# bmds-lab/Crackling

Measured on AMD Instinct MI355X. Metric: guides/sec (whole node) + achieved HBM GB/s, 20bp/<=4mm ISSL scan, higher is better.
Workload: dtype u32

## Files before the change

crackling_amd/csrc/issl_kernels.hip:

```cpp
#include <hip/hip_runtime.h>

#include <algorithm>
#include <type_traits>
#include <cstdio>

#include "issl_device.hpp"

namespace issl {

#define ISSL_CFD_QUAL __constant__
#include "cfd_tables.inc"


__device__ __forceinline__ void short_kernel_priority() { __builtin_amdgcn_s_setprio(3); }

__host__ __device__ inline uint32_t gather_even16(uint32_t x)
{
    x &= 0x55555555u;
    x = (x | (x >> 1)) & 0x33333333u;
    x = (x | (x >> 2)) & 0x0F0F0F0Fu;
    x = (x | (x >> 4)) & 0x00FF00FFu;
    x = (x | (x >> 8)) & 0x0000FFFFu;
    return x;
}
// ... 1657 lines not shown
}

__global__ __launch_bounds__(256) void k_prefix_of_sums(uint32_t *__restrict__ sums, uint32_t n_blocks)
{
    short_kernel_priority();
    __shared__ uint64_t lds[256];
    uint64_t carry = 0;
    for (uint32_t base = 0; base < n_blocks; base += 256) {
        const uint32_t i = base + threadIdx.x;
        const uint64_t val = i < n_blocks ? sums[i] : 0;
        uint64_t total;
        const uint64_t ex = block_exclusive_scan(val, lds, &total);
        if (i < n_blocks) sums[i] = static_cast<uint32_t>(carry + ex);
        carry += total;
    }
}

__global__ __launch_bounds__(256) void k_prefix_apply(const uint32_t *__restrict__ in, uint32_t n,
                                                      const uint32_t *__restrict__ sums, uint32_t *__restrict__ out,
                                                      uint32_t *__restrict__ big, Counters *__restrict__ counters,
                                                      uint32_t slot_hits)
{
    short_kernel_priority();
    __shared__ uint64_t lds[256];
    const uint32_t base = blockIdx.x * kScanChunk + threadIdx.x * 8u;
    uint32_t val[8];
    uint64_t s = 0;
    uint32_t nb = 0;
    for (uint32_t i = 0; i < 8; ++i) {
        const uint32_t c = (base + i < n) ? in[base + i] : 0u;
        nb += c > kReplayLds;
        val[i] = grouped_hits(c, slot_hits);
        s += val[i];
    }
    if (nb != 0u) {
        uint32_t at = atomicAdd(&counters->n_big, nb);
        for (uint32_t i = 0; i < 8; ++i)
            if (base + i < n && in[base + i] > kReplayLds) big[at++] = base + i;
    }
    uint64_t run = block_exclusive_scan(s, lds, nullptr) + sums[blockIdx.x];
    for (uint32_t i = 0; i < 8; ++i) {
        if (base + i < n) out[base + i] = static_cast<uint32_t>(run);
        run += val[i];
    }
}

__global__ __launch_bounds__(1024) void k_prefix_single(const uint32_t *__restrict__ in, uint32_t n,
                                                        uint32_t *__restrict__ out, uint32_t *__restrict__ big,
                                                        Counters *__restrict__ counters, uint32_t slot_hits)
{
    short_kernel_priority();
    if (slot_hits >= kReplayLds && counters->overflowed == 0u) return;
    __shared__ uint32_t wave_sum[16], wave_big[16];
    const uint32_t lane = threadIdx.x & 63u, wave = threadIdx.x >> 6;
    const uint32_t per = ((n + 1023u) / 1024u + 3u) & ~3u;
    const uint32_t i0 = threadIdx.x * per;
    uint32_t s = 0, b = 0;
    for (uint32_t k = 0; k < per; k += 4) {
        const uint32_t i = i0 + k;
        uint4 q = make_uint4(0, 0, 0, 0);
        if (i + 3 < n) q = *reinterpret_cast<const uint4 *>(in + i);
        else { if (i < n) q.x = in[i]; if (i + 1 < n) q.y = in[i + 1]; if (i + 2 < n) q.z = in[i + 2]; }
        s += grouped_hits(q.x, slot_hits) + grouped_hits(q.y, slot_hits) + grouped_hits(q.z, slot_hits) + grouped_hits(q.w, slot_hits);
        b += (q.x > kReplayLds) + (q.y > kReplayLds) + (q.z > kReplayLds) + (q.w > kReplayLds);
    }
    uint32_t x = s, xb = b;
    for (uint32_t d = 1; d < 64; d <<= 1) {
        const uint32_t y = __shfl_up(x, d, 64), yb = __shfl_up(xb, d, 64);
        if (lane >= d) { x += y; xb += yb; }
    }
    if (lane == 63) { wave_sum[wave] = x; wave_big[wave] = xb; }
    __syncthreads();
    uint32_t run = x - s, brun = xb - b;
    for (uint32_t wv = 0; wv < wave; ++wv) { run += wave_sum[wv]; brun += wave_big[wv]; }
    if (threadIdx.x == 1023u) counters->n_big = brun + b;
    for (uint32_t k = 0; k < per; k += 4) {
        const uint32_t i = i0 + k;
        if (i >= n) break;
        uint4 q = make_uint4(0, 0, 0, 0);
        if (i + 3 < n) q = *reinterpret_cast<const uint4 *>(in + i);
        else { q.x = in[i]; if (i + 1 < n) q.y = in[i + 1]; if (i + 2 < n) q.z = in[i + 2]; }
        const uint32_t ex = grouped_hits(q.x, slot_hits), ey = grouped_hits(q.y, slot_hits), ez = grouped_hits(q.z, slot_hits),
                       ew = grouped_hits(q.w, slot_hits);
        const uint4 o = make_uint4(run, run + ex, run + ex + ey, run + ex + ey + ez);
        if (i + 3 < n) *reinterpret_cast<uint4 *>(out + i) = o;
        else { out[i] = o.x; if (i + 1 < n) out[i + 1] = o.y; if (i + 2 < n) out[i + 2] = o.z; }
        run += ex + ey + ez + ew;
        if (q.x > kReplayLds) big[brun++] = i;
        if (q.y > kReplayLds) big[brun++] = i + 1;
        if (q.z > kReplayLds) big[brun++] = i + 2;
        if (q.w > kReplayLds) big[brun++] = i + 3;
    }
}

__global__ __launch_bounds__(kChunkRecs) void k_group_scatter(const uint64_t *__restrict__ raw,
                                                              const uint32_t *__restrict__ raw_used,
                                                              const Counters *__restrict__ counters, uint32_t cap_chunks,
                                                              const uint32_t *__restrict__ gcount,
                                                              const uint32_t *__restrict__ goff,
                                                              const uint32_t *__restrict__ rank,
                                                              const double2 *__restrict__ pay,
                                                              uint64_t *__restrict__ sorted, double2 *__restrict__ terms,
                                                              uint32_t slot_hits)
{
    short_kernel_priority();
    if (slot_hits >= kReplayLds && counters->n_big == 0u) return;
    uint32_t n_chunks = counters->raw_chunks;
    if (n_chunks > cap_chunks) n_chunks = cap_chunks;
    for (uint32_t chunk = blockIdx.x; chunk < n_chunks; chunk += gridDim.x) {
        const uint64_t *recs = raw + static_cast<uint64_t>(chunk) * kChunkRecs;
        const uint32_t t = threadIdx.x + 1u;
        const uint64_t slot = static_cast<uint64_t>(chunk) * (kChunkRecs - 1u) + (threadIdx.x < kChunkRecs - 1u ? threadIdx.x : kChunkRecs - 2u);
        const uint64_t key = recs[t < kChunkRecs ? t : 0u];
        const uint32_t my_rank = rank[slot];
        const double2 my_pay = pay[slot];
        const uint32_t used = raw_used[chunk];
        if (t >= used || t >= kChunkRecs || key == kDeadKey) continue;
        const uint32_t guide = static_cast<uint32_t>(key >> kKeyGuideShift);
        const uint32_t to = goff[guide] + my_rank;
        sorted[to] = key;
        if (gcount[guide] <= kMidHits) terms[to] = my_pay;
    }
}

void launch_group_hits(const Workspace &ws, uint32_t n, void *stream_)
{
    if (ws.lean_tail) return;
    hipStream_t stream = static_cast<hipStream_t>(stream_);
    const uint32_t m = n + 1;
    if (m <= (1u << 18)) {
        hipLaunchKernelGGL(k_prefix_single, dim3(1), dim3(1024), 0, stream, ws.gcount, m, ws.goff, ws.gcur_big,
                           ws.counters, ws.slot_hits);
    } else {
        const uint32_t blocks = (m + kScanChunk - 1) / kScanChunk;
        hipLaunchKernelGGL(k_prefix_block_sums, dim3(blocks), dim3(256), 0, stream, ws.gcount, m, ws.blocksum, ws.slot_hits);
        hipLaunchKernelGGL(k_prefix_of_sums, dim3(1), dim3(256), 0, stream, ws.blocksum, blocks);
        hipLaunchKernelGGL(k_prefix_apply, dim3(blocks), dim3(256), 0, stream, ws.gcount, m, ws.blocksum, ws.goff,
                           ws.gcur_big, ws.counters, ws.slot_hits);
    }
    hipLaunchKernelGGL(k_group_scatter, dim3(kTailGrid), dim3(kChunkRecs), 0, stream, ws.raw, ws.raw_used, ws.counters,
                       static_cast<uint32_t>(ws.cap_chunks), ws.gcount, ws.goff, ws.rank, reinterpret_cast<const double2 *>(ws.pay),
                       ws.sorted, reinterpret_cast<double2 *>(ws.terms), ws.slot_hits);
}



__device__ inline void wave_sort(uint64_t *data, uint32_t n)
{
    if (n < 2) return;
    uint32_t np = 1;
    while (np < n) np <<= 1;
    for (uint32_t k = 2; k <= np; k <<= 1) {
        for (uint32_t j = k >> 1; j > 0; j >>= 1) {
            for (uint32_t t = threadIdx.x; t < (np >> 1); t += blockDim.x) {
                const uint32_t i = ((t & ~(j - 1u)) << 1) | (t & (j - 1u));
                const uint32_t l = (j == (k >> 1)) ? (i ^ (k - 1u)) : (i | j);
                if (l < n) {
                    const uint64_t a = data[i], b = data[l];
                    if (a > b) { data[i] = b; data[l] = a; }
                }
            }
            __syncthreads();
        }
    }
}

__device__ inline double bcast_f64(double x, int lane)
{
    const uint64_t u = __double_as_longlong(x);
    const uint32_t lo = __builtin_amdgcn_readlane(static_cast<uint32_t>(u), lane);
    const uint32_t hi = __builtin_amdgcn_readlane(static_cast<uint32_t>(u >> 32), lane);
    return __longlong_as_double((static_cast<uint64_t>(hi) << 32) | lo);
}

__device__ __forceinline__ bool accumulate_chunk(double mit_term, double cfd_term, uint32_t cnt, const ScoreParams &p,
                                                 uint32_t lane, double &tot_mit, double &tot_cfd, uint32_t &kept,
                                                 const double2 *chunk_lds)
{
    auto passes = [&](double m, double c) {
        if (p.method == ISSL_METHOD_AND) return m > p.maximum_sum && c > p.maximum_sum;
        if (p.method == ISSL_METHOD_OR) return m > p.maximum_sum || c > p.maximum_sum;
        if (p.method == ISSL_METHOD_AVG) return ((m + c) / 2.0) > p.maximum_sum;
        if (p.method == ISSL_METHOD_MIT) return m > p.maximum_sum;
        if (p.method == ISSL_METHOD_CFD) return c > p.maximum_sum;
        return false;
    };
    {
        double tm = tot_mit, tc = tot_cfd;
        for (uint32_t l0 = 0; l0 < cnt; l0 += 8) {
#pragma unroll
            for (uint32_t l = 0; l < 8; ++l) {
                const double2 t = chunk_lds[l0 + l];
                tm += t.x;
                tc += t.y;
            }
        }
        const bool grows = __ballot(lane < cnt && !(mit_term >= 0.0 && cfd_term >= 0.0)) == 0ull;
        if (grows && !passes(tm, tc)) {
            kept += cnt;
            tot_mit = tm;
            tot_cfd = tc;
            return false;
        }
    }
    double tm = tot_mit, tc = tot_cfd, mine_m = 0.0, mine_c = 0.0;
    for (uint32_t l0 = 0; l0 < cnt; l0 += 8) {
#pragma unroll
        for (uint32_t l = 0; l < 8; ++l) {
            const double2 t = chunk_lds[l0 + l];
            tm += t.x;
            tc += t.y;
            if (lane == l0 + l) { mine_m = tm; mine_c = tc; }
        }
    }
    const bool exit_here = passes(mine_m, mine_c);
    const uint64_t exits = __ballot(exit_here && lane < cnt);
    if (exits != 0ull) {
        const int first = __builtin_ctzll(exits);
        kept += static_cast<uint32_t>(first) + 1u;
        tot_mit = bcast_f64(mine_m, first);
        tot_cfd = bcast_f64(mine_c, first);
        return true;
    }
    kept += cnt;
    tot_mit = tm;
    tot_cfd = tc;
    return false;
}

struct HitTerms {
    double mit, cfd;
    issl_hit rec;
};

__device__ inline HitTerms hit_terms(const ImageView &v, uint64_t gsig, uint32_t g, uint64_t key, bool calc_mit,
                                     bool calc_cfd, bool want_id)
{
    HitTerms t;
    t.mit = 0.0;
    t.cfd = 0.0;
    const uint64_t low = (1ull << v.slice_width) - 1ull;
    const uint32_t slice = static_cast<uint32_t>(key >> kKeySliceShift) & kKeySliceMask;
    uint32_t pos = static_cast<uint32_t>(key);
    const uint32_t bucket = (slice << v.slice_width) + static_cast<uint32_t>((gsig >> (v.slice_width * slice)) & low);
    const uint64_t at = v.bucket_start[bucket] + pos;
    uint32_t id = 0, occ;
    uint64_t ot;
    if (v.srec || v.sid) {
        id = pos;
        const uint64_t site = v.sites[id];
        ot = site & kSigMask;
        occ = static_cast<uint32_t>(site >> 40);
        if (occ == kOccSaturated) occ = v.site_occ[id];
        pos = 0;
        if (want_id && v.entries) {
            const uint64_t *list = v.entries + v.bucket_start[bucket];
            uint64_t lo = 0, hi = v.bucket_start[bucket + 1] - v.bucket_start[bucket];
            while (lo < hi) {
                const uint64_t mid = (lo + hi) >> 1;
                if (static_cast<uint32_t>(list[mid]) < id) lo = mid + 1; else hi = mid;
            }
            pos = static_cast<uint32_t>(lo);
        } else if (want_id) {
            const uint32_t *ss = v.sub_start + static_cast<uint64_t>(bucket) * 257u;
            const uint64_t first = static_cast<uint64_t>(v.tile_first[bucket]) * kTileCands;
            for (uint32_t w = 0; w < 256u; ++w) {
                uint32_t lo = ss[w], hi = ss[w + 1];
                const uint32_t s0 = lo;
                while (lo < hi) {
                    const uint32_t mid = (lo + hi) >> 1;
                    const uint32_t there = v.srec ? v.srec[first + mid].id : v.sid[first + mid];
                    if (there < id) lo = mid + 1; else hi = mid;
                }
                pos += lo - s0;
            }
        }
    } else if (v.occ8) {
        ot = candidate_signature(v, bucket, v.tile_first[bucket] + (pos >> 11), pos & (kTileCands - 1u));
        occ = v.occ8[at];
        if (occ == 255u || want_id) {
            const uint64_t e = v.entries[at];
            id = static_cast<uint32_t>(e);
            occ = static_cast<uint32_t>(e >> 32);
        }
    } else {
        const uint64_t e = v.entries[at];
        id = static_cast<uint32_t>(e);
        occ = static_cast<uint32_t>(e >> 32);
        ot = v.esig ? v.esig[at] : v.sites[id];
    }
    int dist;
    score_terms(v, gsig, ot, occ, calc_mit, calc_cfd, t.mit, t.cfd, dist);
    t.rec.guide = g; t.rec.slice = slice; t.rec.pos = pos; t.rec.id = id;
    t.rec.dist = static_cast<uint32_t>(dist); t.rec.occ = occ;
    return t;
}

__global__ __launch_bounds__(64, 8) void k_replay(ImageView v, Workspace ws, const uint64_t *__restrict__ guides,
                                               uint32_t n, ScoreParams p, double *__restrict__ out_mit,
                                               double *__restrict__ out_cfd, uint32_t *__restrict__ out_kept,
                                               issl_hit *__restrict__ out_hits)
{
    short_kernel_priority();
    __shared__ uint64_t keys[kReplayLds];
    __shared__ __attribute__((aligned(16))) double2 ord[64];
    const bool calc_mit = p.method == ISSL_METHOD_MIT || p.method == ISSL_METHOD_AND || p.method == ISSL_METHOD_OR ||
                          p.method == ISSL_METHOD_AVG;
    const bool calc_cfd = p.method == ISSL_METHOD_CFD || p.method == ISSL_METHOD_AND || p.method == ISSL_METHOD_OR ||
                          p.method == ISSL_METHOD_AVG;
    const uint32_t lane = threadIdx.x;
    if (blockIdx.x == 0 && lane == 0 && ws.counters->overflowed != 0u) atomicOr(&ws.sticky[0], ws.lean_tail ? 6u : 4u);

    for (uint32_t g = blockIdx.x; g < n; g += gridDim.x) {
        const uint32_t h = ws.gcount[g];
        if (h > kReplayLds) continue;
        const bool slots = ws.slot_hits >= kReplayLds;
        const uint32_t h0 = slots ? 0u : ws.goff[g];
        const SlotRec *__restrict__ srec = ws.slots + static_cast<uint64_t>(g) * ws.slot_hits;
        const uint64_t *__restrict__ skeys = ws.sorted + h0;
        const double2 *__restrict__ sterms = reinterpret_cast<const double2 *>(ws.terms) + h0;
        auto key_of = [&](uint32_t i) { return slots ? srec[i].key : skeys[i]; };
        auto terms_of = [&](uint32_t i) { return slots ? *reinterpret_cast<const double2 *>(&srec[i].mit) : sterms[i]; };
        const uint64_t gsig = guides[g];
        double tot_mit = 0.0, tot_cfd = 0.0;
        uint32_t kept = 0;
        bool stop = false;

        auto accumulate = [&](double mit_term, double cfd_term, uint32_t cnt) {
            stop = accumulate_chunk(mit_term, cfd_term, cnt, p, lane, tot_mit, tot_cfd, kept, ord);
        };

        if (h <= 64) {
            uint64_t key = ~0ull;
            double2 mine = make_double2(0.0, 0.0);
            issl_hit rec{};
            if (lane < h) {
                key = key_of(lane);
                mine = terms_of(lane);
                if (out_hits) rec = hit_terms(v, gsig, g, key, calc_mit, calc_cfd, true).rec;
            }
            uint32_t rank = 0;
            for (uint32_t j = 0; j < h; ++j) {
                const uint32_t klo = __builtin_amdgcn_readlane(static_cast<uint32_t>(key), static_cast<int>(j));
                const uint32_t khi = __builtin_amdgcn_readlane(static_cast<uint32_t>(key >> 32), static_cast<int>(j));
                const uint64_t other = (static_cast<uint64_t>(khi) << 32) | klo;
                rank += (other < key) ? 1u : 0u;
            }
            if (lane < h) {
                ord[rank] = mine;
                if (out_hits) out_hits[h0 + rank] = rec;
            } else {
                ord[lane] = make_double2(0.0, 0.0);
            }
            __syncthreads();
            const double2 t = ord[lane];
            accumulate(t.x, t.y, h);
        } else {
            uint64_t *data = keys;
            for (uint32_t i = lane; i < h; i += 64) keys[i] = ((key_of(i) & ((1ull << kKeyGuideShift) - 1ull)) << 9) | i;
            __syncthreads();
            wave_sort(data, h);
            __syncthreads();
            for (uint32_t base = 0; base < h && !stop; base += 64) {
                const uint32_t idx = base + lane;
                double2 mine = make_double2(0.0, 0.0);
                if (idx < h) {
                    const uint64_t sv = data[idx];
                    mine = terms_of(static_cast<uint32_t>(sv & 511ull));
                    if (out_hits)
                        out_hits[h0 + idx] = hit_terms(v, gsig, g, (static_cast<uint64_t>(g) << kKeyGuideShift) | (sv >> 9), calc_mit, calc_cfd, true).rec;
                }
                __syncthreads();
                ord[lane] = mine;
                __syncthreads();
                accumulate(mine.x, mine.y, (h - base < 64u) ? h - base : 64u);
            }
        }
        if (lane == 0) {
            out_mit[g] = 10000.0 / (100.0 + tot_mit);
            out_cfd[g] = 10000.0 / (100.0 + tot_cfd);
            if (out_kept) out_kept[g] = kept;
        }
        __syncthreads();
    }
}

constexpr uint32_t kMidSlice = 1024;
constexpr uint32_t kBigSmall = 16384;
constexpr uint32_t kMidDirect = 256;
struct ReplayTicket {
    uint32_t next = 0, turn = 0;
};
__device__ __forceinline__ uint32_t replay_take(ReplayTicket &t, uint32_t *cur , Counters *counters, uint32_t which,
                                                bool first, uint32_t n_entries)
{
    if (n_entries <= gridDim.x) return first ? blockIdx.x : n_entries;
    if (threadIdx.x == 0) {
        if (first) t.next = atomicAdd(&counters->replay_next[which], 1u);
        cur[t.turn] = t.next;
    }
    __syncthreads();
    const uint32_t b = cur[t.turn];
    t.turn ^= 1u;
    if (threadIdx.x == 0) t.next = atomicAdd(&counters->replay_next[which], 1u);
    return b;
}

__global__ __launch_bounds__(256, 6) void k_replay_mid(ImageView v, Workspace ws, const uint64_t *__restrict__ guides,
                                                    ScoreParams p, double *__restrict__ out_mit,
                                                    double *__restrict__ out_cfd, uint32_t *__restrict__ out_kept,
                                                    issl_hit *__restrict__ out_hits)
{
    short_kernel_priority();
    __shared__ __attribute__((aligned(16))) uint32_t head[kMidSlice];
    __shared__ uint16_t head_idx[kMidSlice];
    __shared__ __attribute__((aligned(16))) double2 tmc[kMidSlice];
    __shared__ uint32_t slice_cnt[kMaxSlices];
    __shared__ uint32_t group_at[257], group_cur[256], id_min, id_max;
    __shared__ uint32_t head_fill, stopped_s, carry_kept, cur_entry[2];
    __shared__ double carry_mit, carry_cfd;
    const bool calc_mit = p.method == ISSL_METHOD_MIT || p.method == ISSL_METHOD_AND || p.method == ISSL_METHOD_OR ||
                          p.method == ISSL_METHOD_AVG;
    const bool calc_cfd = p.method == ISSL_METHOD_CFD || p.method == ISSL_METHOD_AND || p.method == ISSL_METHOD_OR ||
                          p.method == ISSL_METHOD_AVG;
    const uint32_t lane = threadIdx.x & 63u;
    const uint32_t n_big = ws.counters->n_big;
    const double2 *__restrict__ terms2 = reinterpret_cast<const double2 *>(ws.terms);
    if (blockIdx.x >= n_big) return;
    ReplayTicket ticket;
    for (bool first = true;; first = false) {
        const uint32_t b = replay_take(ticket, cur_entry, ws.counters, 0u, first, n_big);
        if (b >= n_big) break;
        const uint32_t g = ws.gcur_big[b];
        const uint32_t h = ws.gcount[g];
        if (h > kMidHits) {
            if (threadIdx.x == 0) {
                if (h <= kBigSmall) ws.gcur_big2[atomicAdd(&ws.counters->n_big2, 1u)] = g;
                else ws.gcur_big2[static_cast<uint32_t>(ws.cap_guides) - atomicAdd(&ws.counters->n_big3, 1u)] = g;
            }
            continue;
        }
        const uint32_t h0 = ws.goff[g];
        const uint64_t gsig = guides[g];
        const uint32_t in_slots = ws.slot_hits;
        const SlotRec *__restrict__ srec = ws.slots + static_cast<uint64_t>(g) * in_slots;
        const uint64_t *__restrict__ gkeys = ws.sorted + h0;
        unsigned long long *st = (ws.stamps && b < 4096u) ? ws.stamps + kStampsMid + 16u * b : nullptr;
        if (st && threadIdx.x == 0) { st[0] = __builtin_amdgcn_s_memrealtime(); st[1] = h; st[15] = blockIdx.x; st[14] = 1; }
        if (threadIdx.x < kMaxSlices) slice_cnt[threadIdx.x] = 0;
        if (threadIdx.x == 0) { stopped_s = 0; carry_mit = 0.0; carry_cfd = 0.0; carry_kept = 0; }
        __syncthreads();
        uint64_t mykey[kMidHits / 256];
#pragma unroll
        for (uint32_t k = 0; k < kMidHits / 256; ++k) {
            const uint32_t i = k * 256u + threadIdx.x;
            mykey[k] = i < h ? (i < in_slots ? srec[i].key : gkeys[i]) : ~0ull;
        }
#pragma unroll
        for (uint32_t k = 0; k < kMidHits / 256; ++k) {
            if (k * 256u >= h) break;
            const uint32_t sl = mykey[k] != ~0ull ? static_cast<uint32_t>(mykey[k] >> kKeySliceShift) & kKeySliceMask : kKeySliceMask;
            for (uint32_t s2 = 0; s2 < v.n_slices; ++s2) {
                const uint64_t mm = __ballot(sl == s2);
                if (mm != 0ull && lane == 0) atomicAdd(&slice_cnt[s2], static_cast<uint32_t>(__builtin_popcountll(mm)));
            }
        }
        __syncthreads();
        uint32_t longest = 0;
        for (uint32_t s2 = 0; s2 < v.n_slices; ++s2) longest = slice_cnt[s2] > longest ? slice_cnt[s2] : longest;
        if (longest > kMidSlice) {
            if (threadIdx.x == 0) ws.gcur_big2[atomicAdd(&ws.counters->n_big2, 1u)] = g;
            __syncthreads();
            continue;
        }
        if (st && threadIdx.x == 0) st[2] = __builtin_amdgcn_s_memrealtime();
        uint32_t walked = 0;
        for (uint32_t s2 = 0; s2 < v.n_slices; ++s2) {
            const uint32_t len = slice_cnt[s2];
            if (len == 0) continue;
            const bool grouped_rank = len > kMidDirect;
            if (threadIdx.x == 0) { head_fill = 0; id_min = 0xFFFFFFFFu; id_max = 0u; }
            group_cur[threadIdx.x] = 0;
            __syncthreads();
            uint32_t mn = 0xFFFFFFFFu, mx = 0u;
#pragma unroll
            for (uint32_t k = 0; k < kMidHits / 256; ++k) {
                if (k * 256u >= h) break;
                const uint64_t key = mykey[k];
                const bool mine = key != ~0ull && (static_cast<uint32_t>(key >> kKeySliceShift) & kKeySliceMask) == s2;
                const uint64_t mm = __ballot(mine);
                if (mm == 0ull) continue;
                uint32_t at = 0;
                if (lane == 0) at = atomicAdd(&head_fill, static_cast<uint32_t>(__builtin_popcountll(mm)));
                at = __builtin_amdgcn_readfirstlane(at);
                if (mine) {
                    const uint32_t to = at + __builtin_amdgcn_mbcnt_hi(static_cast<uint32_t>(mm >> 32), __builtin_amdgcn_mbcnt_lo(static_cast<uint32_t>(mm), 0u));
                    const uint32_t id = static_cast<uint32_t>(key);
                    head[to] = id;
                    head_idx[to] = static_cast<uint16_t>(k * 256u + threadIdx.x);
                    mn = id < mn ? id : mn;
                    mx = id > mx ? id : mx;
                }
            }
            if (grouped_rank && mn <= mx) { atomicMin(&id_min, mn); atomicMax(&id_max, mx); }
            __syncthreads();
            auto rank_against_all = [&](auto k_tag) {
                constexpr uint32_t K = decltype(k_tag)::value;
                if (threadIdx.x < 4u && len + threadIdx.x < ((len + 3u) & ~3u)) head[len + threadIdx.x] = 0xFFFFFFFFu;
                __syncthreads();
                uint32_t mine[K], rk[K];
#pragma unroll
                for (uint32_t k = 0; k < K; ++k) { mine[k] = threadIdx.x + k * 256u < len ? head[threadIdx.x + k * 256u] : 0xFFFFFFFFu; rk[k] = 0; }
                const uint4 *quads = reinterpret_cast<const uint4 *>(head);
#pragma unroll 4
                for (uint32_t j = 0; j < (len + 3u) / 4u; ++j) {
                    const uint4 q = quads[j];
#pragma unroll
                    for (uint32_t k = 0; k < K; ++k)
                        rk[k] += (q.x < mine[k] ? 1u : 0u) + (q.y < mine[k] ? 1u : 0u) + (q.z < mine[k] ? 1u : 0u) + (q.w < mine[k] ? 1u : 0u);
                }
#pragma unroll
                for (uint32_t k = 0; k < K; ++k) {
                    if (threadIdx.x + k * 256u >= len) continue;
                    const uint32_t idx = head_idx[threadIdx.x + k * 256u];
                    const double2 t2 = idx < in_slots ? *reinterpret_cast<const double2 *>(&srec[idx].mit) : terms2[h0 + idx];
                    tmc[rk[k]] = t2;
                    if (out_hits)
                        out_hits[h0 + walked + rk[k]] = hit_terms(v, gsig, g, (static_cast<uint64_t>(g) << kKeyGuideShift) |
                                                                      (static_cast<uint64_t>(s2) << kKeySliceShift) | mine[k],
                                                                  calc_mit, calc_cfd, true).rec;
                }
            };
            if (!grouped_rank) {
                rank_against_all(std::integral_constant<uint32_t, 1u>{});
            } else {
                const uint32_t low = id_min, top = id_max - low;
                const uint32_t shift = top < 256u ? 0u : 24u - static_cast<uint32_t>(__builtin_clz(top));
#pragma unroll
                for (uint32_t k = 0; k < kMidSlice / 256; ++k)
                    if (threadIdx.x + k * 256u < len) atomicAdd(&group_cur[(head[threadIdx.x + k * 256u] - low) >> shift], 1u);
                __syncthreads();
                if (threadIdx.x < 64) {
                    uint32_t v4[4], sum = 0, big = 0;
                    for (uint32_t k = 0; k < 4; ++k) { v4[k] = group_cur[threadIdx.x * 4 + k]; sum += v4[k]; big = v4[k] > big ? v4[k] : big; }
                    uint32_t x = sum;
                    for (uint32_t d = 1; d < 64; d <<= 1) {
                        const uint32_t y = __shfl_up(x, d, 64);
                        if (threadIdx.x >= d) x += y;
                    }
                    for (uint32_t d = 32; d > 0; d >>= 1) { const uint32_t y = __shfl_xor(big, d, 64); big = y > big ? y : big; }
                    uint32_t run = x - sum;
                    for (uint32_t k = 0; k < 4; ++k) { group_at[threadIdx.x * 4 + k] = run; group_cur[threadIdx.x * 4 + k] = run; run += v4[k]; }
                    if (threadIdx.x == 63) group_at[256] = run;
                    if (threadIdx.x == 0) id_max = big;
                }
                __syncthreads();
                if (id_max * 4u > len) {
                    if (len <= 512u) rank_against_all(std::integral_constant<uint32_t, 2u>{});
                    else rank_against_all(std::integral_constant<uint32_t, 4u>{});
                } else {
                uint32_t *ids2 = reinterpret_cast<uint32_t *>(tmc);
                uint16_t *idx2 = reinterpret_cast<uint16_t *>(ids2 + kMidSlice);
#pragma unroll
                for (uint32_t k = 0; k < kMidSlice / 256; ++k) {
                    const uint32_t i = threadIdx.x + k * 256u;
                    if (i >= len) continue;
                    const uint32_t id = head[i];
                    const uint32_t to = atomicAdd(&group_cur[(id - low) >> shift], 1u);
                    ids2[to] = id;
                    idx2[to] = head_idx[i];
                }
                if (threadIdx.x < 4u && len + threadIdx.x < ((len + 3u) & ~3u)) ids2[len + threadIdx.x] = 0xFFFFFFFFu;
                __syncthreads();
                const uint4 *quads2 = reinterpret_cast<const uint4 *>(ids2);
#pragma unroll
                for (uint32_t k = 0; k < kMidSlice / 256; ++k) {
                    const uint32_t i = threadIdx.x + k * 256u;
                    if (i < len) {
                        const uint32_t id = ids2[i];
                        const uint32_t g0 = group_at[(id - low) >> shift], g1 = group_at[((id - low) >> shift) + 1u];
                        uint32_t r = g0 & ~3u;
                        for (uint32_t j = g0 >> 2; j < (g1 + 3u) >> 2; ++j) {
                            const uint4 q = quads2[j];
                            r += (q.x < id ? 1u : 0u) + (q.y < id ? 1u : 0u) + (q.z < id ? 1u : 0u) + (q.w < id ? 1u : 0u);
                        }
                        head[r] = id;
                        head_idx[r] = idx2[i];
                    }
                }
                __syncthreads();
#pragma unroll
                for (uint32_t k = 0; k < kMidSlice / 256; ++k) {
                    const uint32_t i = threadIdx.x + k * 256u;
                    if (i < len) {
                        const uint32_t idx = head_idx[i];
                        tmc[i] = idx < in_slots ? *reinterpret_cast<const double2 *>(&srec[idx].mit) : terms2[h0 + idx];
                        if (out_hits)
                            out_hits[h0 + walked + i] = hit_terms(v, gsig, g, (static_cast<uint64_t>(g) << kKeyGuideShift) |
                                                                      (static_cast<uint64_t>(s2) << kKeySliceShift) | head[i],
                                                                  calc_mit, calc_cfd, true).rec;
                    }
                }
                }
            }
            if (threadIdx.x < 8u && len + threadIdx.x < ((len + 7u) & ~7u)) tmc[len + threadIdx.x] = make_double2(0.0, 0.0);
            __syncthreads();
            if (st && threadIdx.x == 0 && walked == 0) { st[3] = __builtin_amdgcn_s_memrealtime(); st[4] = len; }
            if (threadIdx.x < 64) {
                double tot_mit = carry_mit, tot_cfd = carry_cfd;
                uint32_t kept = carry_kept;
                bool stop = false;
                for (uint32_t base = 0; base < len && !stop; base += 64) {
                    const uint32_t idx = base + lane;
                    const double2 mine2 = idx < len ? tmc[idx] : make_double2(0.0, 0.0);
                    stop = accumulate_chunk(mine2.x, mine2.y, (len - base < 64u) ? len - base : 64u, p, lane, tot_mit, tot_cfd, kept,
                                            tmc + base);
                }
                if (lane == 0) { carry_mit = tot_mit; carry_cfd = tot_cfd; carry_kept = kept; stopped_s = stop ? 1u : 0u; }
            }
            __syncthreads();
            walked += len;
            if (stopped_s != 0u) break;
        }
        if (threadIdx.x == 0) {
            out_mit[g] = 10000.0 / (100.0 + carry_mit);
            out_cfd[g] = 10000.0 / (100.0 + carry_cfd);
            if (out_kept) out_kept[g] = carry_kept;
            if (st) { st[7] = __builtin_amdgcn_s_memrealtime(); st[8] = carry_kept; st[9] = walked; }
        }
        __syncthreads();
    }
}

template <uint32_t K, uint32_t THREADS>
__device__ __forceinline__ void rank_sort_slice(const uint32_t *pos_lds, uint32_t len, uint64_t high_bits,
                                                uint64_t *__restrict__ dst)
{
    uint32_t mine[K], rk[K];
#pragma unroll
    for (uint32_t k = 0; k < K; ++k) {
        const uint32_t idx = threadIdx.x + k * THREADS;
        mine[k] = idx < len ? pos_lds[idx] : 0xFFFFFFFFu;
        rk[k] = 0;
    }
    const uint4 *quads = reinterpret_cast<const uint4 *>(pos_lds);
    const uint32_t n_quads = (len + 3u) >> 2;
#pragma unroll 4
    for (uint32_t j = 0; j < n_quads; ++j) {
        const uint4 q = quads[j];
#pragma unroll
        for (uint32_t k = 0; k < K; ++k)
            rk[k] += (q.x < mine[k] ? 1u : 0u) + (q.y < mine[k] ? 1u : 0u) + (q.z < mine[k] ? 1u : 0u) +
                     (q.w < mine[k] ? 1u : 0u);
    }
#pragma unroll
    for (uint32_t k = 0; k < K; ++k)
        if (threadIdx.x + k * THREADS < len) dst[rk[k]] = high_bits | mine[k];
}

__device__ __forceinline__ void rank_sort_slice_grouped(const uint32_t *pos_lds, uint32_t *grouped, uint32_t *group_at ,
                                                        uint32_t *group_cur , uint32_t *max_pos, uint32_t *min_pos,
                                                        uint32_t len, uint64_t high_bits, uint64_t *__restrict__ dst)
{
    if (threadIdx.x < 256) group_cur[threadIdx.x] = 0;
    if (threadIdx.x == 0) { *max_pos = 0; *min_pos = 0xFFFFFFFFu; }
    __syncthreads();
    uint32_t m = 0, mn = 0xFFFFFFFFu;
    for (uint32_t i = threadIdx.x; i < len; i += blockDim.x) { const uint32_t q = pos_lds[i]; m = q > m ? q : m; mn = q < mn ? q : mn; }
    atomicMax(max_pos, m);
    atomicMin(min_pos, mn);
    __syncthreads();
    const uint32_t low = *min_pos, top = *max_pos - low;
    const uint32_t shift = top < 256u ? 0u : 24u - static_cast<uint32_t>(__builtin_clz(top));
// ... 270 lines not shown
```

Measured before the change: 42.12 million.

## Replace wave sort in replay with per-slice counting rank when slices are short

In k_replay's large-hit path, hits are now bucketed by slice using wave ballots, laid out per slice in LDS, and each hit's rank is computed by comparing its id against the other ids in the same slice with vectorized uint4 LDS reads. The result is written into a 16-bit permutation array. This replaces the general wave_sort of 64-bit keys whenever no slice holds more than 128 hits, and falls back to wave_sort otherwise. It is meant to cut sorting cost for guides with many hits, at the price of more register state (eight slice-position slots per lane) and reuse of the LDS buffer for several tables. The output order relies on slice-then-id ordering matching the original key order.

```diff
diff --git a/crackling_amd/csrc/issl_kernels.hip b/crackling_amd/csrc/issl_kernels.hip
--- a/crackling_amd/csrc/issl_kernels.hip
+++ b/crackling_amd/csrc/issl_kernels.hip
@@ -1983,7 +1983,7 @@
                                                issl_hit *__restrict__ out_hits)
 {
     short_kernel_priority();
-    __shared__ uint64_t keys[kReplayLds];
+    __shared__ __attribute__((aligned(16))) uint64_t keys[kReplayLds];
     __shared__ __attribute__((aligned(16))) double2 ord[64];
     const bool calc_mit = p.method == ISSL_METHOD_MIT || p.method == ISSL_METHOD_AND || p.method == ISSL_METHOD_OR ||
                           p.method == ISSL_METHOD_AVG;
@@ -2037,19 +2037,85 @@
             const double2 t = ord[lane];
             accumulate(t.x, t.y, h);
         } else {
-            uint64_t *data = keys;
-            for (uint32_t i = lane; i < h; i += 64) keys[i] = ((key_of(i) & ((1ull << kKeyGuideShift) - 1ull)) << 9) | i;
-            __syncthreads();
-            wave_sort(data, h);
+            constexpr uint32_t kRankSlice = 128;
+            const uint32_t rounds = (h + 63u) / 64u;
+            uint32_t sp[8];
+            uint32_t cnt = 0;
+#pragma unroll
+            for (uint32_t r = 0; r < 8; ++r) {
+                sp[r] = 0u;
+                if (r >= rounds) continue;
+                const bool valid = lane + 64u * r < h;
+                uint64_t key = 0ull;
+                if (valid) key = key_of(lane + 64u * r);
+                const uint32_t sl = static_cast<uint32_t>(key >> kKeySliceShift) & kKeySliceMask;
+                for (uint64_t left = __ballot(valid); left != 0ull;) {
+                    const uint32_t s = __builtin_amdgcn_readlane(sl, __builtin_ctzll(left));
+                    const bool in = valid && sl == s;
+                    const uint64_t m = __ballot(in);
+                    const uint32_t before = __builtin_amdgcn_readlane(cnt, static_cast<int>(s));
+                    if (in) sp[r] = (s << 16) | (before + __builtin_amdgcn_mbcnt_hi(static_cast<uint32_t>(m >> 32),
+                                                                                    __builtin_amdgcn_mbcnt_lo(static_cast<uint32_t>(m), 0u)));
+                    if (lane == s) cnt += static_cast<uint32_t>(__builtin_popcountll(m));
+                    left &= ~m;
+                }
+            }
+            uint32_t off = 0, first = 0, longest = 0;
+            {
+                uint32_t po = 0, pr = 0;
+                for (uint32_t s = 0; s < v.n_slices; ++s) {
+                    const uint32_t c = __builtin_amdgcn_readlane(cnt, static_cast<int>(s));
+                    if (lane == s) { off = po; first = pr; }
+                    po += (c + 3u) & ~3u;
+                    pr += c;
+                    longest = c > longest ? c : longest;
+                }
+            }
+            uint32_t *ids = reinterpret_cast<uint32_t *>(keys);
+            uint16_t *perm = reinterpret_cast<uint16_t *>(ids + kReplayLds + 4u * kMaxSlices);
+            uint32_t *tab = ids + kReplayLds + 4u * kMaxSlices + kReplayLds / 2u;
+            static_assert((kReplayLds + 4u * kMaxSlices + kReplayLds / 2u + 3u * kMaxSlices) * 4u <= sizeof(uint64_t) * kReplayLds,
+                          "k_replay LDS");
+            const bool counted = longest <= kRankSlice;
+            if (counted) {
+                if (lane < v.n_slices) {
+                    const uint32_t padded = (cnt + 3u) & ~3u;
+                    for (uint32_t k = cnt; k < padded; ++k) ids[off + k] = ~0u;
+                    tab[lane] = off; tab[kMaxSlices + lane] = first; tab[2u * kMaxSlices + lane] = padded;
+                }
+                __syncthreads();
+#pragma unroll
+                for (uint32_t r = 0; r < 8; ++r)
+                    if (r < rounds && lane + 64u * r < h)
+                        ids[tab[sp[r] >> 16] + (sp[r] & 0xFFFFu)] = static_cast<uint32_t>(key_of(lane + 64u * r));
+                __syncthreads();
+#pragma unroll
+                for (uint32_t r = 0; r < 8; ++r) {
+                    if (r < rounds && lane + 64u * r < h) {
+                        const uint32_t s = sp[r] >> 16, len = tab[2u * kMaxSlices + s], at = tab[s];
+                        const uint32_t id = ids[at + (sp[r] & 0xFFFFu)];
+                        uint32_t rank = tab[kMaxSlices + s];
+                        const uint4 *q4 = reinterpret_cast<const uint4 *>(ids + at);
+                        for (uint32_t j = 0; j < len / 4u; ++j) {
+                            const uint4 q = q4[j];
+                            rank += (q.x < id) + (q.y < id) + (q.z < id) + (q.w < id);
+                        }
+                        perm[rank] = static_cast<uint16_t>(lane + 64u * r);
+                    }
+                }
+            } else {
+                for (uint32_t i = lane; i < h; i += 64) keys[i] = ((key_of(i) & ((1ull << kKeyGuideShift) - 1ull)) << 9) | i;
+                __syncthreads();
+                wave_sort(keys, h);
+            }
             __syncthreads();
             for (uint32_t base = 0; base < h && !stop; base += 64) {
                 const uint32_t idx = base + lane;
                 double2 mine = make_double2(0.0, 0.0);
                 if (idx < h) {
-                    const uint64_t sv = data[idx];
-                    mine = terms_of(static_cast<uint32_t>(sv & 511ull));
-                    if (out_hits)
-                        out_hits[h0 + idx] = hit_terms(v, gsig, g, (static_cast<uint64_t>(g) << kKeyGuideShift) | (sv >> 9), calc_mit, calc_cfd, true).rec;
+                    const uint32_t src = counted ? perm[idx] : static_cast<uint32_t>(keys[idx] & 511ull);
+                    mine = terms_of(src);
+                    if (out_hits) out_hits[h0 + idx] = hit_terms(v, gsig, g, key_of(src), calc_mit, calc_cfd, true).rec;
                 }
                 __syncthreads();
                 ord[lane] = mine;
```

Result: faster. 42.65 million, median of 6 (+1.3%).
